# aerius-labs/indexed-merkle-tree-halo2

Measured on AMD Instinct MI355X. Metric: indexed-tree insertions/sec at depth=32 (bn256::Fr), higher is better.
Workload: dtype u32 limbs (9 x 29-bit, Montgomery mod p), 64-bit accumulate

## Files before the change

indexed-merkle-tree-halo2_amd/csrc/imt_consts.hpp:

```cpp
#pragma once
#include <cstdint>

namespace imt {
namespace dev {

constexpr int NL = 9;
constexpr uint32_t MASK29 = (1u << 29) - 1;

struct Fe {
    uint32_t v[NL];
};

constexpr int RF = 8, RP = 57;
struct PoseidonConsts {
    Fe rc_full[RF][3];
    Fe rc_h2p2[3];
    Fe k_partial[RP];
    Fe mats[2][3][3];
    Fe sp_row[RP][3];
    Fe sp_col[RP][2];
    Fe sp_gamma[RP];
    Fe cap0;
    Fe one;
    Fe from_canon;
    Fe from_mont256;
    Fe to_mont256;
    Fe int_one;
    Fe zero_leaf;
};

struct TraceConsts {
    Fe absorb[3][3];
    Fe full_c[RF][3];
    Fe partial[RP];
    Fe mats[2][3][3];
    Fe row[RP][3];
    Fe col_hat[RP][2];
};
constexpr int TRACE_ROWS_H2 = 1208, TRACE_ROWS_H3 = 1209;

}
}
```

indexed-merkle-tree-halo2_amd/csrc/imt_coop_device.hpp:

```cpp
#pragma once
#if !defined(__HIP_DEVICE_COMPILE__)
#error "device-only header"
#endif
#include <cstddef>
#include "imt_device.hpp"

namespace imt {
namespace dev {
namespace coop {

constexpr unsigned TAB_DWORDS = sizeof(PoseidonConsts) / 4;
#define IMT_COOP_E(member) ((unsigned)(offsetof(PoseidonConsts, member) / sizeof(Fe)))

__device__ __forceinline__ void tab_fill(uint32_t* tab, const PoseidonConsts& pc) {
    const uint32_t* src = reinterpret_cast<const uint32_t*>(&pc);
    for (unsigned i = threadIdx.x; i < TAB_DWORDS; i += blockDim.x) tab[i] = src[i];
    __syncthreads();
}
__device__ __forceinline__ void tab_fe(Fe& r, const uint32_t* tab, unsigned entry) {
#pragma unroll
    for (int i = 0; i < NL; i++) r.v[i] = tab[entry * NL + i];
}
template <int J>
__device__ __forceinline__ void quad_bcast(Fe& r, const Fe& x) {
#pragma unroll
    for (int i = 0; i < NL; i++) r.v[i] = (uint32_t)__builtin_amdgcn_mov_dpp((int)x.v[i], J * 0x55, 0xf, 0xf, true);
}
__device__ __forceinline__ void sel(Fe& r, bool c, const Fe& a, const Fe& b) {
#pragma unroll
    for (int i = 0; i < NL; i++) r.v[i] = c ? a.v[i] : b.v[i];
}

__device__ __forceinline__ void permute(const uint32_t* tab, Fe& S, unsigned ri, unsigned first_rc) {
    const bool is0 = ri == 0;
#pragma unroll 1
    for (int st = 0; st < RF + RP; st++) {
        if (st < RF / 2 || st >= RF / 2 + RP) {
            const int f = st < RF / 2 ? st : st - RP;
            Fe k, v, x2, x4, y, Y[3], M[3];
            tab_fe(k, tab, (st == 0 ? first_rc : IMT_COOP_E(rc_full) + 3u * (unsigned)f) + ri);
            add_lazy(v, S, k);
            masm::sqr_v_narrow(x2, v);
            masm::sqr_v_narrow(x4, x2);
            masm::mul_vv_narrow(y, &x4, &v);
            quad_bcast<0>(Y[0], y);
// ... 57 lines not shown
```

indexed-merkle-tree-halo2_amd/csrc/imt_device.hpp:

```cpp
#pragma once
#include <cstddef>
#include <cstdint>
#include "imt_consts.hpp"

#if defined(__HIPCC__)
#include <hip/hip_runtime.h>
#define IMT_HD __host__ __device__ __forceinline__
#else
#define IMT_HD inline
#endif

namespace imt {
namespace dev {

#define IMT_P29_0 0x10000001u
#define IMT_P29_1 0x1f0fac9fu
#define IMT_P29_2 0x0e5c2450u
#define IMT_P29_3 0x07d090f3u
#define IMT_P29_4 0x1585d283u
#define IMT_P29_5 0x02db40c0u
#define IMT_P29_6 0x00a6e141u
#define IMT_P29_7 0x0e5c2634u
#define IMT_P29_8 0x0030644eu
constexpr uint32_t N0INV29 = 0x0fffffffu;
// ... 158 lines not shown
    for (int i = 0; i < NL; i++) {
        uint32_t d = a.v[i] - p29(i) - borrow;
        borrow = (i < NL - 1) ? (d >> 31) : 0;
        a.v[i] = (i < NL - 1) ? (d & MASK29) : d;
    }
}

template <int SH>
IMT_HD constexpr uint32_t p29_shl(int i) {
    return i == 0 ? ((p29(0) << SH) & MASK29)
         : i < NL - 1 ? (((p29(i) << SH) | (p29(i - 1) >> (29 - SH))) & MASK29)
                      : ((p29(i) << SH) | (p29(i - 1) >> (29 - SH)));
}
template <int SH>
IMT_HD void cond_sub_p_shl(Fe& a) {
    bool ge = true;
#pragma unroll
    for (int i = 0; i < NL; i++) {
        const uint32_t pi = p29_shl<SH>(i);
        if (a.v[i] != pi) ge = a.v[i] > pi;
    }
    if (ge) {
        uint32_t borrow = 0;
#pragma unroll
        for (int i = 0; i < NL; i++) {
            uint32_t d = a.v[i] - p29_shl<SH>(i) - borrow;
            borrow = (i < NL - 1) ? (d >> 31) : 0;
            a.v[i] = (i < NL - 1) ? (d & MASK29) : d;
        }
    }
}

IMT_HD void canonicalize(Fe& a) {
    cond_sub_p_shl<3>(a);
    cond_sub_p_shl<2>(a);
    cond_sub_p_shl<1>(a);
    cond_sub_p_shl<0>(a);
}

IMT_HD void unpack(Fe& r, const uint32_t w[8]) {
#pragma unroll
    for (int i = 0; i < NL; i++) {
        const int bit = 29 * i, wi = bit >> 5, sh = bit & 31;
        uint32_t lo = w[wi] >> sh;
        if (sh > 3 && wi + 1 < 8) lo |= w[wi + 1] << (32 - sh);
        r.v[i] = lo & MASK29;
    }
}
IMT_HD void pack(uint32_t w[8], const Fe& a) {
#pragma unroll
    for (int j = 0; j < 8; j++) {
        const int lo_limb = (32 * j) / 29, off = 32 * j - 29 * lo_limb;
        uint32_t x = a.v[lo_limb] >> off;
        const int have = 29 - off;
        if (have < 32 && lo_limb + 1 < NL) x |= a.v[lo_limb + 1] << have;
        if (have + 29 < 32 && lo_limb + 2 < NL) x |= a.v[lo_limb + 2] << (have + 29);
        w[j] = x;
    }
}

struct alignas(16) Word4 { uint32_t x, y, z, w; };
IMT_HD void load_packed(Fe& r, const void* ptr) {
    const Word4* q = reinterpret_cast<const Word4*>(ptr);
    Word4 x = q[0], y = q[1];
    uint32_t w[8] = {x.x, x.y, x.z, x.w, y.x, y.y, y.z, y.w};
    unpack(r, w);
}
IMT_HD void store_packed(void* ptr, const Fe& a) {
    uint32_t w[8];
    pack(w, a);
    Word4* q = reinterpret_cast<Word4*>(ptr);
    q[0] = Word4{w[0], w[1], w[2], w[3]};
    q[1] = Word4{w[4], w[5], w[6], w[7]};
}



IMT_HD void sbox(Fe& x) {
    Fe x2, x4;
    mont_sqr(x2, x);
    mont_sqr(x4, x2);
    mont_mul(x, x4, x);
}

IMT_HD void permute(const PoseidonConsts& pc, Fe s[3], const Fe* first_rc) {
    constexpr int NSTEP = RF + (RP + 1) / 2;
#pragma unroll 1
    for (int st = 0; st < NSTEP; st++) {
        if (st < RF / 2 || st >= RF / 2 + (RP + 1) / 2) {
            const int fr = st < RF / 2 ? st : st - (RP + 1) / 2;
            const Fe* rc = (st == 0) ? first_rc : pc.rc_full[fr];
            add_lazy(s[0], s[0], rc[0]);
            add_lazy(s[1], s[1], rc[1]);
            add_lazy(s[2], s[2], rc[2]);
            sbox(s[0]); sbox(s[1]); sbox(s[2]);
            const Fe(*mat)[3] = pc.mats[st == RF / 2 - 1 ? 1 : 0];
            Fe n0, n1, n2;
            mont_dot_uc<3, false>(n0, mat[0], s, s[0]);
            mont_dot_uc<3, false>(n1, mat[1], s, s[0]);
            mont_dot_uc<3, false>(n2, mat[2], s, s[0]);
            s[0] = n0; s[1] = n1; s[2] = n2;
        } else {
            const int p = 2 * (st - RF / 2);
            const bool second = p + 1 < RP;
            Fe v[4], y[2], n0;
            add_lazy(v[0], s[0], pc.k_partial[p]);
            sbox(v[0]);
            v[1] = s[1]; v[2] = s[2];
            mont_dot_uc<3, false>(n0, pc.sp_row[p], v, v[0]);
            y[0] = v[0];
#pragma unroll
            for (int i = 0; i < NL; i++) y[1].v[i] = 0;
            if (second) {
                add_lazy(v[0], n0, pc.k_partial[p + 1]);
                sbox(v[0]);
                v[3] = y[0];
                const Fe c4[4] = {pc.sp_row[p + 1][0], pc.sp_row[p + 1][1], pc.sp_row[p + 1][2], pc.sp_gamma[p + 1]};
                mont_dot_uc<4, false>(n0, c4, v, v[0]);
                y[1] = v[0];
            }
            const int q = second ? p + 1 : p;
            const Fe c1[2] = {pc.sp_col[p][0], pc.sp_col[q][0]};
            const Fe c2[2] = {pc.sp_col[p][1], pc.sp_col[q][1]};
            mont_dot_uc<2, true, false>(s[1], c1, y, s[1]);
            mont_dot_uc<2, true, false>(s[2], c2, y, s[2]);
            s[0] = n0;
        }
    }
}

IMT_HD void hash23(const PoseidonConsts& pc, Fe& out, const Fe& a, const Fe& b, const Fe& c, bool three) {
    Fe s[3] = {pc.cap0, a, b};
#pragma unroll 1
    for (int blk = 0; blk < 2; blk++) {
        const Fe* rc0 = pc.rc_full[0];
        if (blk == 1) {
            if (three) {
                add_lazy(s[1], s[1], c);
                add_lazy(s[2], s[2], pc.one);
                normalize(s[1]);
                normalize(s[2]);
            } else {
                rc0 = pc.rc_h2p2;
            }
        }
        permute(pc, s, rc0);
    }
    out = s[1];
    canonicalize(out);
}
IMT_HD void hash23_stashed(const PoseidonConsts& pc, Fe& out, const Fe& a, const Fe& b, bool three,
                           const uint32_t* stash, unsigned stride) {
    Fe s[3] = {pc.cap0, a, b};
#pragma unroll 1
    for (int blk = 0; blk < 2; blk++) {
        const Fe* rc0 = pc.rc_full[0];
        if (blk == 1) {
            if (three) {
// ... 54 lines not shown
```

indexed-merkle-tree-halo2_amd/csrc/imt_flags.hip:

```cpp
#include <hip/hip_runtime.h>
#include <algorithm>
#include "imt_flags.hpp"

namespace {

__global__ void k_flag_set(uint64_t* flag, uint64_t value) {
    if (threadIdx.x == 0 && blockIdx.x == 0) __hip_atomic_store(flag, value, __ATOMIC_RELEASE, __HIP_MEMORY_SCOPE_SYSTEM);
}

__device__ inline bool poisoned(const uint32_t* poison) {
    return poison && __hip_atomic_load(poison, __ATOMIC_RELAXED, __HIP_MEMORY_SCOPE_SYSTEM) != 0;
}

__global__ void k_flag_set_checked(uint64_t* flag, uint64_t value, const uint32_t* poison) {
    if (threadIdx.x == 0 && blockIdx.x == 0 && !poisoned(poison)) __hip_atomic_store(flag, value, __ATOMIC_RELEASE, __HIP_MEMORY_SCOPE_SYSTEM);
}

__global__ void k_flag_wait(imt::launch::FlagWait w) {
    if (threadIdx.x != 0 || blockIdx.x != 0) return;
    if (poisoned(w.err)) return;
    const uint64_t t0 = wall_clock64();
    for (int i = 0; i < w.n; i++) {
        while (__hip_atomic_load(w.flag[i], __ATOMIC_ACQUIRE, __HIP_MEMORY_SCOPE_SYSTEM) < w.value) {
            if (wall_clock64() - t0 > w.timeout_ticks) {
                __hip_atomic_fetch_or(w.err, 1u << (i & 31), __ATOMIC_RELAXED, __HIP_MEMORY_SCOPE_SYSTEM);
                return;
            }
            __builtin_amdgcn_s_sleep(64);
        }
    }
}

__global__ void k_copy16(uint4* __restrict__ dst, const uint4* __restrict__ src, size_t n16, const uint32_t* poison) {
    if (poisoned(poison)) return;
    for (size_t i = (size_t)blockIdx.x * blockDim.x + threadIdx.x; i < n16; i += (size_t)gridDim.x * blockDim.x) dst[i] = src[i];
}

__global__ void k_copy16_multi(imt::launch::CopyJobs jobs, size_t n16, const uint32_t* poison) {
    if (poisoned(poison)) return;
    uint4* __restrict__ dst = (uint4*)jobs.dst[blockIdx.y];
    const uint4* __restrict__ src = (const uint4*)jobs.src[blockIdx.y];
    for (size_t i = (size_t)blockIdx.x * blockDim.x + threadIdx.x; i < n16; i += (size_t)gridDim.x * blockDim.x) dst[i] = src[i];
}

__global__ void k_spin(uint64_t ticks, uint64_t* end_stamp) {
    if (threadIdx.x != 0 || blockIdx.x != 0) return;
    const uint64_t t0 = wall_clock64();
    while (wall_clock64() - t0 < ticks) __builtin_amdgcn_s_sleep(32);
    *end_stamp = wall_clock64();
}
__global__ void k_stamp(uint64_t* stamp) {
    if (threadIdx.x == 0 && blockIdx.x == 0) *stamp = wall_clock64();
}

}

namespace imt {
namespace launch {

void copy16(hipStream_t s, void* dst, const void* src, size_t bytes, const uint32_t* poison) {
    const size_t n16 = bytes / 16;
    if (!n16) return;
    const unsigned blocks = (unsigned)std::min<size_t>((n16 + 255) / 256, 512);
    hipLaunchKernelGGL(k_copy16, dim3(blocks), dim3(256), 0, s, (uint4*)dst, (const uint4*)src, n16, poison);
}

void copy16_multi(hipStream_t s, const CopyJobs& jobs, size_t bytes, const uint32_t* poison) {
    const size_t n16 = bytes / 16;
    if (!n16 || jobs.n <= 0) return;
    const unsigned blocks = (unsigned)std::min<size_t>((n16 + 255) / 256, 64);
    hipLaunchKernelGGL(k_copy16_multi, dim3(blocks, (unsigned)jobs.n), dim3(256), 0, s, jobs, n16, poison);
}

void flag_set_checked(hipStream_t s, uint64_t* flag, uint64_t value, const uint32_t* poison) {
    hipLaunchKernelGGL(k_flag_set_checked, dim3(1), dim3(64), 0, s, flag, value, poison);
}

void spin(hipStream_t s, uint64_t ticks, uint64_t* end_stamp) { hipLaunchKernelGGL(k_spin, dim3(1), dim3(64), 0, s, ticks, end_stamp); }
void stamp(hipStream_t s, uint64_t* out) { hipLaunchKernelGGL(k_stamp, dim3(1), dim3(64), 0, s, out); }

void flag_set(hipStream_t s, uint64_t* flag, uint64_t value) { hipLaunchKernelGGL(k_flag_set, dim3(1), dim3(64), 0, s, flag, value); }

void flag_wait(hipStream_t s, const FlagWait& w) {
    if (w.n > 0) hipLaunchKernelGGL(k_flag_wait, dim3(1), dim3(64), 0, s, w);
}

}
}
```

indexed-merkle-tree-halo2_amd/csrc/imt_flags.hpp:

```cpp
#pragma once
#include <hip/hip_runtime_api.h>
#include <cstdint>

namespace imt {
namespace launch {

constexpr int FLAG_WAIT_MAX = 16;
struct FlagWait {
    const uint64_t* flag[FLAG_WAIT_MAX];
    int n;
    uint64_t value;
    uint64_t timeout_ticks;
    uint32_t* err;
};
void flag_set(hipStream_t s, uint64_t* flag, uint64_t value);
void flag_wait(hipStream_t s, const FlagWait& w);
void copy16(hipStream_t s, void* dst, const void* src, size_t bytes, const uint32_t* poison = nullptr);
struct CopyJobs {
    void* dst[FLAG_WAIT_MAX];
    const void* src[FLAG_WAIT_MAX];
    int n;
};
void copy16_multi(hipStream_t s, const CopyJobs& jobs, size_t bytes, const uint32_t* poison);
void flag_set_checked(hipStream_t s, uint64_t* flag, uint64_t value, const uint32_t* poison);
void spin(hipStream_t s, uint64_t ticks, uint64_t* end_stamp);
void stamp(hipStream_t s, uint64_t* out);

}
}
```

indexed-merkle-tree-halo2_amd/csrc/imt_fr_host.hpp:

```cpp
#pragma once
#include <cstdint>
#include <cstring>

namespace imt {

typedef unsigned __int128 u128;

struct HFr {
    uint64_t l[4];
    bool operator==(const HFr& o) const { return std::memcmp(l, o.l, 32) == 0; }
};

struct HField {
    static constexpr uint64_t P[4] = {0x43e1f593f0000001ULL, 0x2833e84879b97091ULL,
                                      0xb85045b68181585dULL, 0x30644e72e131a029ULL};
    uint64_t inv;
    HFr r1, r2;
    HFr r3;

    HField() {
        uint64_t x = 1;
        for (int i = 0; i < 7; i++) x *= 2 - P[0] * x;
        inv = 0 - x;
        uint64_t t[4] = {1, 0, 0, 0};
// ... 66 lines not shown
        for (int i = 0; i < 4; i++) {
            uint64_t m = t[i] * inv;
            u128 c = 0;
            for (int j = 0; j < 4; j++) {
                c += (u128)m * P[j] + t[i + j];
                t[i + j] = (uint64_t)c;
                c >>= 64;
            }
            for (int k = i + 4; k < 9 && c; k++) {
                c += t[k];
                t[k] = (uint64_t)c;
                c >>= 64;
            }
        }
        HFr o;
        std::memcpy(o.l, t + 4, 32);
        if (t[8] || geq_p(o.l)) sub_p(o.l);
        return o;
    }
    HFr from_u64(uint64_t v) const { return mul(HFr{{v, 0, 0, 0}}, r2); }
    HFr zero() const { return HFr{{0, 0, 0, 0}}; }
    HFr one() const { return r1; }
    bool from_bytes(HFr& out, const uint8_t in[32]) const {
        HFr t;
        std::memcpy(t.l, in, 32);
        if (geq_p(t.l)) return false;
        out = mul(t, r2);
        return true;
    }
    void to_bytes(uint8_t out[32], const HFr& a) const {
        HFr t = mul(a, HFr{{1, 0, 0, 0}});
        std::memcpy(out, t.l, 32);
    }
    HFr inverse(const HFr& a) const {
        uint64_t e[4] = {P[0] - 2, P[1], P[2], P[3]};
        HFr acc = r1, base = a;
        for (int i = 0; i < 256; i++) {
            if ((e[i / 64] >> (i % 64)) & 1) acc = mul(acc, base);
            base = mul(base, base);
        }
        return acc;
    }
    bool is_zero(const HFr& a) const { return (a.l[0] | a.l[1] | a.l[2] | a.l[3]) == 0; }
};

inline int cmp_le32(const uint8_t* a, const uint8_t* b) {
    const uint64_t* x = reinterpret_cast<const uint64_t*>(a);
    const uint64_t* y = reinterpret_cast<const uint64_t*>(b);
    uint64_t xa[4], ya[4];
    std::memcpy(xa, x, 32);
    std::memcpy(ya, y, 32);
    for (int i = 3; i >= 0; i--) {
        if (xa[i] != ya[i]) return xa[i] < ya[i] ? -1 : 1;
    }
    return 0;
}

}
```

indexed-merkle-tree-halo2_amd/csrc/imt_params.cpp:

```cpp
#include "imt_params.hpp"

namespace imt {

namespace {
struct Grain {
    uint8_t b[80];
    int pos = 0;
    int new_bit() {
        int p = pos;
        auto g = [&](int k) { return b[(p + k) % 80]; };
        int nb = g(62) ^ g(51) ^ g(38) ^ g(23) ^ g(13) ^ g(0);
        b[p] = (uint8_t)nb;
        pos = (p + 1) % 80;
        return nb;
    }
    int next() {
        while (!new_bit()) new_bit();
        return new_bit();
    }
    void take254(uint8_t le[32]) {
        std::memset(le, 0, 32);
        for (int i = 253; i >= 0; i--)
            if (next()) le[i / 8] |= (uint8_t)(1u << (i % 8));
    }
// ... 20 lines not shown

void HostPoseidon::permute_opt(HFr s[3]) const {
    auto sbox = [&](HFr& x) {
        HFr x2 = F.mul(x, x), x4 = F.mul(x2, x2);
        x = F.mul(x4, x);
    };
    auto dense = [&](const HFr m[3][3]) {
        HFr n[3];
        for (int i = 0; i < 3; i++) {
            n[i] = F.mul(m[i][0], s[0]);
            n[i] = F.add(n[i], F.mul(m[i][1], s[1]));
            n[i] = F.add(n[i], F.mul(m[i][2], s[2]));
        }
        s[0] = n[0]; s[1] = n[1]; s[2] = n[2];
    };
    for (int r = 0; r < 65; r++) {
        if (r < 4 || r >= 61) {
            const int fr = r < 4 ? r : r - 57;
            for (int i = 0; i < 3; i++) s[i] = F.add(s[i], rc_full[fr][i]);
            for (int i = 0; i < 3; i++) sbox(s[i]);
            dense(r == 3 ? pre : mds);
        } else {
            const int p = r - 4;
            HFr y = F.add(s[0], k_partial[p]);
            sbox(y);
            HFr n0 = F.mul(sp_row[p][0], y);
            n0 = F.add(n0, F.mul(sp_row[p][1], s[1]));
            n0 = F.add(n0, F.mul(sp_row[p][2], s[2]));
            s[1] = F.add(s[1], F.mul(sp_col[p][0], y));
            s[2] = F.add(s[2], F.mul(sp_col[p][1], y));
            s[0] = n0;
        }
    }
}

void HostPoseidon::permute_spec(HFr s[3]) const {
    auto x5c = [&](HFr& x, const HFr& c) {
        HFr x2 = F.mul(x, x), x4 = F.mul(x2, x2);
        x = F.add(F.mul(x4, x), c);
    };
    auto dense = [&](const HFr m[3][3]) {
        HFr n[3];
        for (int i = 0; i < 3; i++) {
            n[i] = F.mul(m[i][0], s[0]);
            n[i] = F.add(n[i], F.mul(m[i][1], s[1]));
            n[i] = F.add(n[i], F.mul(m[i][2], s[2]));
        }
        s[0] = n[0]; s[1] = n[1]; s[2] = n[2];
    };
    for (int i = 0; i < 3; i++) s[i] = F.add(s[i], tr_start[0][i]);
    for (int r = 1; r <= 4; r++) {
        for (int i = 0; i < 3; i++) x5c(s[i], tr_start[r][i]);
        dense(r == 4 ? tr_pre : mds);
    }
    for (int p = 0; p < 57; p++) {
        x5c(s[0], tr_partial[p]);
        HFr n0 = F.mul(tr_row[p][0], s[0]);
        n0 = F.add(n0, F.mul(tr_row[p][1], s[1]));
        n0 = F.add(n0, F.mul(tr_row[p][2], s[2]));
        s[1] = F.add(F.mul(tr_col_hat[p][0], s[0]), s[1]);
        s[2] = F.add(F.mul(tr_col_hat[p][1], s[0]), s[2]);
        s[0] = n0;
    }
    for (int r = 0; r < 4; r++) {
        for (int i = 0; i < 3; i++) x5c(s[i], r < 3 ? tr_end[r][i] : F.zero());
        dense(mds);
// ... 66 lines not shown
        HFr mw[3];
        matvec(mds, w, mw);
        for (int i = 0; i < 3; i++) rc_full[4][i] = F.add(rc[61][i], mw[i]);
    }
    for (int r = 62; r < 65; r++)
        for (int i = 0; i < 3; i++) rc_full[r - 57][i] = rc[r][i];

    HFr cur[3][3];
    std::memcpy(cur, mds, sizeof cur);
    for (int p = 60; p >= 4; p--) {
        HFr det = F.sub(F.mul(cur[1][1], cur[2][2]), F.mul(cur[1][2], cur[2][1]));
        if (F.is_zero(det)) { err = "singular MDS sub-block"; return false; }
        HFr di = F.inverse(det);
        HFr Dinv[2][2] = {{F.mul(cur[2][2], di), F.mul(F.sub(F.zero(), cur[1][2]), di)},
                          {F.mul(F.sub(F.zero(), cur[2][1]), di), F.mul(cur[1][1], di)}};
        sp_row[p - 4][0] = cur[0][0];
        sp_row[p - 4][1] = F.add(F.mul(cur[0][1], Dinv[0][0]), F.mul(cur[0][2], Dinv[1][0]));
        sp_row[p - 4][2] = F.add(F.mul(cur[0][1], Dinv[0][1]), F.mul(cur[0][2], Dinv[1][1]));
        sp_col[p - 4][0] = cur[1][0];
        sp_col[p - 4][1] = cur[2][0];
        HFr np[3][3] = {{F.one(), F.zero(), F.zero()},
                        {F.zero(), cur[1][1], cur[1][2]},
                        {F.zero(), cur[2][1], cur[2][2]}};
        HFr nxt[3][3];
        for (int i = 0; i < 3; i++)
            for (int j = 0; j < 3; j++) {
                nxt[i][j] = F.mul(np[i][0], mds[0][j]);
                nxt[i][j] = F.add(nxt[i][j], F.mul(np[i][1], mds[1][j]));
                nxt[i][j] = F.add(nxt[i][j], F.mul(np[i][2], mds[2][j]));
            }
        std::memcpy(cur, nxt, sizeof cur);
    }
    std::memcpy(pre, cur, sizeof pre);

    {
        typedef HFr M3[3][3];
        auto mat_mul = [&](const M3 a, const M3 b, M3 o) {
            HFr r[3][3];
            for (int i = 0; i < 3; i++)
                for (int j = 0; j < 3; j++) {
                    r[i][j] = F.mul(a[i][0], b[0][j]);
                    r[i][j] = F.add(r[i][j], F.mul(a[i][1], b[1][j]));
                    r[i][j] = F.add(r[i][j], F.mul(a[i][2], b[2][j]));
                }
            std::memcpy(o, r, sizeof r);
        };
        HFr minv[3][3];
        {
            auto cof = [&](int r0, int r1, int c0, int c1) {
                return F.sub(F.mul(mds[r0][c0], mds[r1][c1]), F.mul(mds[r0][c1], mds[r1][c0]));
            };
            HFr adj[3][3];
            for (int i = 0; i < 3; i++)
                for (int j = 0; j < 3; j++) {
                    const int r0 = (j + 1) % 3, r1 = (j + 2) % 3, c0 = (i + 1) % 3, c1 = (i + 2) % 3;
                    adj[i][j] = cof(r0, r1, c0, c1);
                }
            HFr det = F.add(F.add(F.mul(mds[0][0], adj[0][0]), F.mul(mds[0][1], adj[1][0])), F.mul(mds[0][2], adj[2][0]));
            if (F.is_zero(det)) { err = "singular MDS"; return false; }
            HFr di = F.inverse(det);
            for (int i = 0; i < 3; i++)
                for (int j = 0; j < 3; j++) minv[i][j] = F.mul(adj[i][j], di);
        }
        for (int i = 0; i < 3; i++) tr_start[0][i] = rc[0][i];
        for (int r = 1; r < 4; r++) matvec(minv, rc[r], tr_start[r]);
        HFr acc[3] = {rc[61][0], rc[61][1], rc[61][2]};
        for (int p = 56; p >= 0; p--) {
            HFr tmp[3];
            matvec(minv, acc, tmp);
            tr_partial[p] = tmp[0];
            acc[0] = rc[4 + p][0];
            acc[1] = F.add(tmp[1], rc[4 + p][1]);
            acc[2] = F.add(tmp[2], rc[4 + p][2]);
        }
        matvec(minv, acc, tr_start[4]);
        for (int r = 0; r < 3; r++) matvec(minv, rc[62 + r], tr_end[r]);
        HFr mt[3][3], a[3][3];
        for (int i = 0; i < 3; i++)
            for (int j = 0; j < 3; j++) mt[i][j] = a[i][j] = mds[j][i];
        for (int k = 0; k < 57; k++) {
            const int p = 56 - k;
            HFr det = F.sub(F.mul(a[1][1], a[2][2]), F.mul(a[1][2], a[2][1]));
            if (F.is_zero(det)) { err = "singular MDS minor"; return false; }
            HFr di = F.inverse(det);
            HFr hi[2][2] = {{F.mul(a[2][2], di), F.mul(F.sub(F.zero(), a[1][2]), di)},
                            {F.mul(F.sub(F.zero(), a[2][1]), di), F.mul(a[1][1], di)}};
            tr_row[p][0] = a[0][0];
            tr_row[p][1] = F.add(F.mul(hi[0][0], a[1][0]), F.mul(hi[0][1], a[2][0]));
            tr_row[p][2] = F.add(F.mul(hi[1][0], a[1][0]), F.mul(hi[1][1], a[2][0]));
            tr_col_hat[p][0] = a[0][1];
            tr_col_hat[p][1] = a[0][2];
            HFr prime[3][3] = {{F.one(), F.zero(), F.zero()}, {F.zero(), a[1][1], a[1][2]}, {F.zero(), a[2][1], a[2][2]}};
            mat_mul(mt, prime, a);
        }
        for (int i = 0; i < 3; i++)
            for (int j = 0; j < 3; j++) tr_pre[i][j] = a[j][i];
    }

    for (uint64_t t = 0; t < 4; t++) {
        HFr a[3] = {F.from_u64(t * 7919), F.from_u64(t * t + 1), F.mul(cap0, F.from_u64(t + 3))};
        HFr b[3] = {a[0], a[1], a[2]};
        permute_plain(a);
        permute_opt(b);
        if (!(a[0] == b[0] && a[1] == b[1] && a[2] == b[2])) {
            err = "optimised Poseidon schedule disagrees with the plain form";
            return false;
        }
        HFr c3[3] = {F.from_u64(t * 7919), F.from_u64(t * t + 1), F.mul(cap0, F.from_u64(t + 3))};
        permute_spec(c3);
        if (!(a[0] == c3[0] && a[1] == c3[1] && a[2] == c3[2])) {
            err = "halo2-base form of the Poseidon schedule disagrees with the plain form";
            return false;
        }
    }
    return true;
}

void HostPoseidon::fill_trace_consts(dev::TraceConsts& tc) const {
    for (int i = 0; i < 3; i++) {
        tc.absorb[0][i] = to_dev(tr_start[0][i]);
        tc.absorb[1][i] = to_dev(i == 2 ? F.add(tr_start[0][i], F.one()) : tr_start[0][i]);
        tc.absorb[2][i] = to_dev(i == 1 ? F.add(tr_start[0][i], F.one()) : tr_start[0][i]);
    }
    for (int f = 0; f < 8; f++)
        for (int i = 0; i < 3; i++)
            tc.full_c[f][i] = to_dev(f < 4 ? tr_start[f + 1][i] : f < 7 ? tr_end[f - 4][i] : F.zero());
    for (int p = 0; p < 57; p++) {
        tc.partial[p] = to_dev(tr_partial[p]);
        for (int i = 0; i < 3; i++) tc.row[p][i] = to_dev(tr_row[p][i]);
        for (int i = 0; i < 2; i++) tc.col_hat[p][i] = to_dev(tr_col_hat[p][i]);
    }
    for (int i = 0; i < 3; i++)
        for (int j = 0; j < 3; j++) {
            tc.mats[0][i][j] = to_dev(mds[i][j]);
            tc.mats[1][i][j] = to_dev(tr_pre[i][j]);
        }
}

dev::Fe HostPoseidon::int_to_dev_limbs(const uint8_t le[32]) const {
    dev::Fe o;
    for (int i = 0; i < dev::NL; i++) {
        uint32_t v = 0;
        for (int k = 0; k < 29; k++) {
            int bit = 29 * i + k;
            if (bit < 256 && ((le[bit / 8] >> (bit % 8)) & 1)) v |= 1u << k;
        }
        o.v[i] = v;
    }
    return o;
}

dev::Fe HostPoseidon::to_dev(const HFr& x) const {
    HFr two29 = F.from_u64(1ULL << 29);
    HFr t = x;
    for (int i = 0; i < 9; i++) t = F.mul(t, two29);
    uint8_t le[32];
    F.to_bytes(le, t);
    return int_to_dev_limbs(le);
}

void HostPoseidon::fill_consts(dev::PoseidonConsts& pc) const {
    for (int r = 0; r < 8; r++)
        for (int i = 0; i < 3; i++) pc.rc_full[r][i] = to_dev(rc_full[r][i]);
    pc.rc_h2p2[0] = to_dev(rc_full[0][0]);
    pc.rc_h2p2[1] = to_dev(F.add(rc_full[0][1], F.one()));
    pc.rc_h2p2[2] = to_dev(rc_full[0][2]);
    pc.sp_gamma[0] = to_dev(F.zero());
    for (int p = 1; p < 57; p++)
        pc.sp_gamma[p] = to_dev(F.add(F.mul(sp_row[p][1], sp_col[p - 1][0]), F.mul(sp_row[p][2], sp_col[p - 1][1])));
    for (int p = 0; p < 57; p++) {
        pc.k_partial[p] = to_dev(k_partial[p]);
        for (int i = 0; i < 3; i++) pc.sp_row[p][i] = to_dev(sp_row[p][i]);
        for (int i = 0; i < 2; i++) pc.sp_col[p][i] = to_dev(sp_col[p][i]);
    }
    for (int i = 0; i < 3; i++)
        for (int j = 0; j < 3; j++) {
            pc.mats[0][i][j] = to_dev(mds[i][j]);
            pc.mats[1][i][j] = to_dev(pre[i][j]);
        }
    pc.cap0 = to_dev(cap0);
    pc.one = to_dev(F.one());
    HFr two29 = F.from_u64(1ULL << 29), r261 = F.one();
    for (int i = 0; i < 9; i++) r261 = F.mul(r261, two29);
    HFr two64 = cap0, two256 = F.mul(F.mul(two64, two64), F.mul(two64, two64));
    uint8_t le[32];
    auto as_int = [&](const HFr& x) { F.to_bytes(le, x); return int_to_dev_limbs(le); };
    pc.from_canon = as_int(F.mul(r261, r261));
    pc.from_mont256 = as_int(F.mul(F.mul(r261, r261), F.inverse(two256)));
    pc.to_mont256 = as_int(two256);
    std::memset(le, 0, 32); le[0] = 1;
    pc.int_one = int_to_dev_limbs(le);
    HFr z = F.zero();
    pc.zero_leaf = to_dev(hash3(z, z, z));
}

}
```

indexed-merkle-tree-halo2_amd/csrc/imt_params.hpp:

```cpp
#pragma once
#include "imt_consts.hpp"
#include "imt_fr_host.hpp"
#include <string>
#include <vector>

namespace imt {

struct HostPoseidon {
    HField F;
    HFr rc[65][3];
    HFr mds[3][3];
    HFr rc_full[8][3];
    HFr k_partial[57];
    HFr pre[3][3];
    HFr sp_row[57][3];
    HFr sp_col[57][2];
    HFr cap0;
    HFr tr_start[5][3], tr_partial[57], tr_end[3][3];
    HFr tr_pre[3][3];
    HFr tr_row[57][3], tr_col_hat[57][2];

    bool init(std::string& err);

    void permute_plain(HFr s[3]) const;
    void permute_opt(HFr s[3]) const;
    void permute_spec(HFr s[3]) const;
    void fill_trace_consts(dev::TraceConsts& tc) const;
    HFr hash2(const HFr& a, const HFr& b) const;
    HFr hash3(const HFr& a, const HFr& b, const HFr& c) const;

    dev::Fe to_dev(const HFr& x) const;
    dev::Fe int_to_dev_limbs(const uint8_t le[32]) const;
    void fill_consts(dev::PoseidonConsts& pc) const;
};

}
```

indexed-merkle-tree-halo2_amd/csrc/imt_sliced.cpp:

```cpp
#include <fcntl.h>
#include <sys/mman.h>
#include <sys/stat.h>
#include <unistd.h>
#include <algorithm>
#include <atomic>
#include <chrono>
#include <condition_variable>
#include <deque>
#include <mutex>
#include <cstdio>
#include <cstring>
#include <memory>
#include <new>
#include <string>
#include <thread>
#include <vector>
#include "imt_flags.hpp"
#include "imt_itree_internal.hpp"
#include "imt_sliced_sched.hpp"
#include "imt_sliced_transport.hpp"

using namespace imt::sliced;

namespace {
// ... 60 lines not shown
        }
    };
    env("IMT_SLICED_COMM_STREAMS", IMT_SLICED_OPT_COMM_STREAMS, o);
    env("IMT_SLICED_COMM_PRIO", IMT_SLICED_OPT_COMM_PRIORITY, o);
    env("IMT_SLICED_ROUND_PRIO", IMT_SLICED_OPT_ROUND_PRIORITIES, o);
    env("IMT_SLICED_APPLY_STREAMS", IMT_SLICED_OPT_APPLY_STREAMS, o);
    env("IMT_SLICED_PREP_STREAM", IMT_SLICED_OPT_PREP_STREAM, o);
    env("IMT_SLICED_VERIFY_QUEUES", IMT_SLICED_OPT_VERIFY_QUEUES, o);
    env("IMT_SLICED_WATCHDOG_MS", IMT_SLICED_OPT_WATCHDOG_MS, o);
    env("IMT_SLICED_TIMING", IMT_SLICED_OPT_TIMING, o);
    env("IMT_SLICED_COMM_PLACEMENT", IMT_SLICED_OPT_COMM_PLACEMENT, o);
    env("IMT_SLICED_POOLS", IMT_SLICED_OPT_POOLS, o);
    return o;
}

template <class Query>
int bounded_wait(imt_ctx* ctx, long limit_ms, Query query, const char* what) {
    const auto t0 = std::chrono::steady_clock::now();
    for (unsigned spins = 0;; spins++) {
        const hipError_t e = query();
        if (e == hipSuccess) return IMT_OK;
        if (e != hipErrorNotReady) return ctx->hip_fail(e, what);
        if (spins > 2000) std::this_thread::sleep_for(std::chrono::microseconds(50));
        if (limit_ms > 0 && (spins & 63) == 63 &&
            std::chrono::duration<double, std::milli>(std::chrono::steady_clock::now() - t0).count() > (double)limit_ms)
            return ctx->fail(IMT_ERR_TIMEOUT, "gave up after %ld ms waiting for %s (IMT_SLICED_OPT_WATCHDOG_MS)", limit_ms, what);
    }
}

struct QueueProbe {
    imt_ctx* ctx = nullptr;
    uint64_t* d = nullptr;
    static constexpr int MAXS = 16;
    uint64_t spin_ticks = 20000;
    int probes = 0;

    int init(imt_ctx* c) {
        ctx = c;
        int khz = 100000;
        if (hipDeviceGetAttribute(&khz, hipDeviceAttributeWallClockRate, c->device) != hipSuccess || khz <= 0) khz = 100000;
        spin_ticks = (uint64_t)khz / 5;
        IMT_HIP(c, hipMalloc((void**)&d, sizeof(uint64_t) * (MAXS + 1)));
        imt::launch::spin(c->stream, 1, d + MAXS);
        imt::launch::stamp(c->stream, d);
        IMT_HIP(c, hipStreamSynchronize(c->stream));
        return IMT_OK;
    }
    ~QueueProbe() {
        if (d) hipFree(d);
    }
    int run(hipStream_t busy, const hipStream_t* others, int n, char* behind) {
        if (n > MAXS) return ctx->fail(IMT_ERR_INTERNAL, "queue probe: too many streams");
        uint64_t h[MAXS + 1];
        IMT_HIP(ctx, hipStreamSynchronize(busy));
        for (int j = 0; j < n; j++) IMT_HIP(ctx, hipStreamSynchronize(others[j]));
        IMT_HIP(ctx, hipMemsetAsync(d, 0, sizeof(uint64_t) * (MAXS + 1), ctx->stream));
        IMT_HIP(ctx, hipStreamSynchronize(ctx->stream));
        imt::launch::spin(busy, spin_ticks, d + MAXS);
        for (int j = 0; j < n; j++) imt::launch::stamp(others[j], d + j);
        IMT_HIP(ctx, hipGetLastError());
        IMT_HIP(ctx, hipStreamSynchronize(busy));
        for (int j = 0; j < n; j++) IMT_HIP(ctx, hipStreamSynchronize(others[j]));
        IMT_HIP(ctx, hipMemcpy(h, d, sizeof h, hipMemcpyDeviceToHost));
        for (int j = 0; j < n; j++) behind[j] = h[j] >= h[MAXS];
        probes++;
        return IMT_OK;
    }
};

struct HipBackend : Backend {
    imt_itree* tree;
    imt_ctx* ctx;
    hipStream_t rs[ROUNDS] = {}, cs[ROUNDS] = {}, aps[ROUNDS] = {};
    int n_comm = ROUNDS;
    int round_prio = 0;
    SlicedOptions opt;
    int q_round[ROUNDS], q_comm[ROUNDS], q_apply[ROUNDS];
    int n_queues = 0, placement = IMT_SLICED_PLACEMENT_UNVERIFIED, streams_recreated = 0;
    bool comm_own_queues = false;
    bool hung = false;
    std::string placement_note;

    explicit HipBackend(imt_itree* t) : tree(t), ctx(imt_itree_ctx(t)) {
        for (int i = 0; i < ROUNDS; i++) q_round[i] = q_comm[i] = q_apply[i] = -1;
    }
    int new_stream(hipStream_t* out, int prio) {
        IMT_HIP(ctx, hipStreamCreateWithPriority(out, hipStreamNonBlocking, prio));
        return IMT_OK;
    }
    void adopt(hipStream_t s) { ctx->side_streams.push_back(s); }
    int init(const SlicedOptions& o, int channels) {
        opt = o;
// ... 1146 lines not shown
```

Baseline: 3.018 million.

## Rescale Poseidon constants by fifth roots to turn multiplies into additions

Precomputes fifth-root diagonal rescalings of the Poseidon state on the host, so that row 0 of most full-round matrices becomes (1,1,1) and one sparse-column coefficient becomes 1. The device permute then uses additions instead of Montgomery dot products for those entries, with a periodic fold to keep the lazily reduced limbs bounded and an extra canonicalize step. The queue probe is also changed to end its spin once all stamp kernels have run, which cuts probe wait time while raising the maximum spin. The rescaled path is checked against the plain schedule on extra inputs, but the lazy-reduction bounds are a correctness risk.

```diff
diff --git a/indexed-merkle-tree-halo2_amd/csrc/imt_consts.hpp b/indexed-merkle-tree-halo2_amd/csrc/imt_consts.hpp
--- a/indexed-merkle-tree-halo2_amd/csrc/imt_consts.hpp
+++ b/indexed-merkle-tree-halo2_amd/csrc/imt_consts.hpp
@@ -19,7 +19,6 @@
     Fe mats[2][3][3];
     Fe sp_row[RP][3];
     Fe sp_col[RP][2];
-    Fe sp_gamma[RP];
     Fe cap0;
     Fe one;
     Fe from_canon;
@@ -27,6 +26,12 @@
     Fe to_mont256;
     Fe int_one;
     Fe zero_leaf;
+    Fe sc_rc[RF][3];
+    Fe sc_mats[RF][3][3];
+    Fe sc_k[RP];
+    Fe sc_row[RP][3];
+    Fe sc_gamma[RP];
+    Fe sc_u[RP];
 };
 
 struct TraceConsts {
diff --git a/indexed-merkle-tree-halo2_amd/csrc/imt_coop_device.hpp b/indexed-merkle-tree-halo2_amd/csrc/imt_coop_device.hpp
--- a/indexed-merkle-tree-halo2_amd/csrc/imt_coop_device.hpp
+++ b/indexed-merkle-tree-halo2_amd/csrc/imt_coop_device.hpp
@@ -9,8 +9,9 @@
 namespace dev {
 namespace coop {
 
-constexpr unsigned TAB_DWORDS = sizeof(PoseidonConsts) / 4;
+constexpr unsigned TAB_DWORDS = offsetof(PoseidonConsts, sc_rc) / 4;
 #define IMT_COOP_E(member) ((unsigned)(offsetof(PoseidonConsts, member) / sizeof(Fe)))
+static_assert(TAB_DWORDS * 4 <= 16236, "the coop kernels' LDS table must not grow");
 
 __device__ __forceinline__ void tab_fill(uint32_t* tab, const PoseidonConsts& pc) {
     const uint32_t* src = reinterpret_cast<const uint32_t*>(&pc);
diff --git a/indexed-merkle-tree-halo2_amd/csrc/imt_device.hpp b/indexed-merkle-tree-halo2_amd/csrc/imt_device.hpp
--- a/indexed-merkle-tree-halo2_amd/csrc/imt_device.hpp
+++ b/indexed-merkle-tree-halo2_amd/csrc/imt_device.hpp
@@ -214,6 +214,7 @@
 }
 
 IMT_HD void canonicalize(Fe& a) {
+    cond_sub_p_shl<4>(a);
     cond_sub_p_shl<3>(a);
     cond_sub_p_shl<2>(a);
     cond_sub_p_shl<1>(a);
@@ -265,47 +266,68 @@
     mont_mul(x, x4, x);
 }
 
+IMT_HD constexpr uint32_t pc29(int i) { return i == 0 ? (1u << 29) - p29(0) : MASK29 - p29(i); }
+constexpr uint32_t FOLD_RECIP = 1354;
+
+IMT_HD void fold_p(Fe& a) {
+    const uint32_t q = (uint32_t)(((uint64_t)a.v[NL - 1] * FOLD_RECIP) >> 32);
+    uint64_t acc = 0;
+#pragma unroll
+    for (int i = 0; i < NL; i++) {
+        acc = (acc >> 29) + a.v[i] + (uint64_t)q * pc29(i);
+        a.v[i] = i < NL - 1 ? (uint32_t)acc & MASK29 : (uint32_t)(acc - ((uint64_t)q << 29));
+    }
+}
+
 IMT_HD void permute(const PoseidonConsts& pc, Fe s[3], const Fe* first_rc) {
     constexpr int NSTEP = RF + (RP + 1) / 2;
 #pragma unroll 1
     for (int st = 0; st < NSTEP; st++) {
         if (st < RF / 2 || st >= RF / 2 + (RP + 1) / 2) {
             const int fr = st < RF / 2 ? st : st - (RP + 1) / 2;
-            const Fe* rc = (st == 0) ? first_rc : pc.rc_full[fr];
+            const Fe* rc = (st == 0) ? first_rc : pc.sc_rc[fr];
             add_lazy(s[0], s[0], rc[0]);
             add_lazy(s[1], s[1], rc[1]);
             add_lazy(s[2], s[2], rc[2]);
             sbox(s[0]); sbox(s[1]); sbox(s[2]);
-            const Fe(*mat)[3] = pc.mats[st == RF / 2 - 1 ? 1 : 0];
+            const Fe(*mat)[3] = pc.sc_mats[fr];
             Fe n0, n1, n2;
-            mont_dot_uc<3, false>(n0, mat[0], s, s[0]);
+            if (fr == 0 || fr == RF / 2) {
+                mont_dot_uc<3, false>(n0, mat[0], s, s[0]);
+            } else {
+                add_lazy(n0, s[0], s[1]);
+                add_lazy(n0, n0, s[2]);
+                normalize(n0);
+            }
             mont_dot_uc<3, false>(n1, mat[1], s, s[0]);
             mont_dot_uc<3, false>(n2, mat[2], s, s[0]);
             s[0] = n0; s[1] = n1; s[2] = n2;
         } else {
             const int p = 2 * (st - RF / 2);
             const bool second = p + 1 < RP;
-            Fe v[4], y[2], n0;
-            add_lazy(v[0], s[0], pc.k_partial[p]);
+            Fe v[4], z[2], n0;
+            add_lazy(v[0], s[0], pc.sc_k[p]);
             sbox(v[0]);
             v[1] = s[1]; v[2] = s[2];
-            mont_dot_uc<3, false>(n0, pc.sp_row[p], v, v[0]);
-            y[0] = v[0];
-#pragma unroll
-            for (int i = 0; i < NL; i++) y[1].v[i] = 0;
+            mont_dot_uc<3, false>(n0, pc.sc_row[p], v, v[0]);
+            z[0] = v[0];
+#pragma unroll
+            for (int i = 0; i < NL; i++) z[1].v[i] = 0;
             if (second) {
-                add_lazy(v[0], n0, pc.k_partial[p + 1]);
+                add_lazy(v[0], n0, pc.sc_k[p + 1]);
                 sbox(v[0]);
-                v[3] = y[0];
-                const Fe c4[4] = {pc.sp_row[p + 1][0], pc.sp_row[p + 1][1], pc.sp_row[p + 1][2], pc.sp_gamma[p + 1]};
+                v[3] = z[0];
+                const Fe c4[4] = {pc.sc_row[p + 1][0], pc.sc_row[p + 1][1], pc.sc_row[p + 1][2], pc.sc_gamma[p + 1]};
                 mont_dot_uc<4, false>(n0, c4, v, v[0]);
-                y[1] = v[0];
+                z[1] = v[0];
             }
             const int q = second ? p + 1 : p;
-            const Fe c1[2] = {pc.sp_col[p][0], pc.sp_col[q][0]};
-            const Fe c2[2] = {pc.sp_col[p][1], pc.sp_col[q][1]};
-            mont_dot_uc<2, true, false>(s[1], c1, y, s[1]);
-            mont_dot_uc<2, true, false>(s[2], c2, y, s[2]);
+            const Fe cu[2] = {pc.sc_u[p], pc.sc_u[q]};
+            mont_dot_uc<2, true, false>(s[2], cu, z, s[2]);
+            add_lazy(s[1], s[1], z[0]);
+            add_lazy(s[1], s[1], z[1]);
+            normalize(s[1]);
+            if ((p & 7) == 6) fold_p(s[1]);
             s[0] = n0;
         }
     }
diff --git a/indexed-merkle-tree-halo2_amd/csrc/imt_flags.hip b/indexed-merkle-tree-halo2_amd/csrc/imt_flags.hip
--- a/indexed-merkle-tree-halo2_amd/csrc/imt_flags.hip
+++ b/indexed-merkle-tree-halo2_amd/csrc/imt_flags.hip
@@ -43,14 +43,18 @@
     for (size_t i = (size_t)blockIdx.x * blockDim.x + threadIdx.x; i < n16; i += (size_t)gridDim.x * blockDim.x) dst[i] = src[i];
 }
 
-__global__ void k_spin(uint64_t ticks, uint64_t* end_stamp) {
+__global__ void k_spin(uint64_t ticks, uint64_t* end_stamp, const uint64_t* count, uint64_t n) {
     if (threadIdx.x != 0 || blockIdx.x != 0) return;
     const uint64_t t0 = wall_clock64();
-    while (wall_clock64() - t0 < ticks) __builtin_amdgcn_s_sleep(32);
+    while (wall_clock64() - t0 < ticks && __hip_atomic_load(count, __ATOMIC_ACQUIRE, __HIP_MEMORY_SCOPE_AGENT) < n)
+        __builtin_amdgcn_s_sleep(32);
     *end_stamp = wall_clock64();
 }
-__global__ void k_stamp(uint64_t* stamp) {
-    if (threadIdx.x == 0 && blockIdx.x == 0) *stamp = wall_clock64();
+__global__ void k_stamp(uint64_t* stamp, uint64_t* count) {
+    if (threadIdx.x == 0 && blockIdx.x == 0) {
+        *stamp = wall_clock64();
+        __hip_atomic_fetch_add(count, (uint64_t)1, __ATOMIC_RELEASE, __HIP_MEMORY_SCOPE_AGENT);
+    }
 }
 
 }
@@ -76,8 +80,10 @@
     hipLaunchKernelGGL(k_flag_set_checked, dim3(1), dim3(64), 0, s, flag, value, poison);
 }
 
-void spin(hipStream_t s, uint64_t ticks, uint64_t* end_stamp) { hipLaunchKernelGGL(k_spin, dim3(1), dim3(64), 0, s, ticks, end_stamp); }
-void stamp(hipStream_t s, uint64_t* out) { hipLaunchKernelGGL(k_stamp, dim3(1), dim3(64), 0, s, out); }
+void spin(hipStream_t s, uint64_t ticks, uint64_t* end_stamp, const uint64_t* count, uint64_t n) {
+    hipLaunchKernelGGL(k_spin, dim3(1), dim3(64), 0, s, ticks, end_stamp, count, n);
+}
+void stamp(hipStream_t s, uint64_t* out, uint64_t* count) { hipLaunchKernelGGL(k_stamp, dim3(1), dim3(64), 0, s, out, count); }
 
 void flag_set(hipStream_t s, uint64_t* flag, uint64_t value) { hipLaunchKernelGGL(k_flag_set, dim3(1), dim3(64), 0, s, flag, value); }
 
diff --git a/indexed-merkle-tree-halo2_amd/csrc/imt_flags.hpp b/indexed-merkle-tree-halo2_amd/csrc/imt_flags.hpp
--- a/indexed-merkle-tree-halo2_amd/csrc/imt_flags.hpp
+++ b/indexed-merkle-tree-halo2_amd/csrc/imt_flags.hpp
@@ -23,8 +23,8 @@
 };
 void copy16_multi(hipStream_t s, const CopyJobs& jobs, size_t bytes, const uint32_t* poison);
 void flag_set_checked(hipStream_t s, uint64_t* flag, uint64_t value, const uint32_t* poison);
-void spin(hipStream_t s, uint64_t ticks, uint64_t* end_stamp);
-void stamp(hipStream_t s, uint64_t* out);
+void spin(hipStream_t s, uint64_t ticks, uint64_t* end_stamp, const uint64_t* count, uint64_t n);
+void stamp(hipStream_t s, uint64_t* out, uint64_t* count);
 
 }
 }
diff --git a/indexed-merkle-tree-halo2_amd/csrc/imt_fr_host.hpp b/indexed-merkle-tree-halo2_amd/csrc/imt_fr_host.hpp
--- a/indexed-merkle-tree-halo2_amd/csrc/imt_fr_host.hpp
+++ b/indexed-merkle-tree-halo2_amd/csrc/imt_fr_host.hpp
@@ -122,14 +122,33 @@
         HFr t = mul(a, HFr{{1, 0, 0, 0}});
         std::memcpy(out, t.l, 32);
     }
-    HFr inverse(const HFr& a) const {
-        uint64_t e[4] = {P[0] - 2, P[1], P[2], P[3]};
+    HFr pow(const HFr& a, const uint64_t e[4]) const {
         HFr acc = r1, base = a;
         for (int i = 0; i < 256; i++) {
             if ((e[i / 64] >> (i % 64)) & 1) acc = mul(acc, base);
             base = mul(base, base);
         }
         return acc;
+    }
+    HFr inverse(const HFr& a) const {
+        const uint64_t e[4] = {P[0] - 2, P[1], P[2], P[3]};
+        return pow(a, e);
+    }
+    HFr fifth_root(const HFr& a) const {
+        uint64_t e[4];
+        u128 c = 1;
+        for (int i = 0; i < 4; i++) {
+            c += (u128)P[i] * 4 - (i == 0 ? 4 : 0);
+            e[i] = (uint64_t)c;
+            c >>= 64;
+        }
+        u128 rem = 0;
+        for (int i = 3; i >= 0; i--) {
+            u128 cur = (rem << 64) | e[i];
+            e[i] = (uint64_t)(cur / 5);
+            rem = cur % 5;
+        }
+        return pow(a, e);
     }
     bool is_zero(const HFr& a) const { return (a.l[0] | a.l[1] | a.l[2] | a.l[3]) == 0; }
 };
diff --git a/indexed-merkle-tree-halo2_amd/csrc/imt_params.cpp b/indexed-merkle-tree-halo2_amd/csrc/imt_params.cpp
--- a/indexed-merkle-tree-halo2_amd/csrc/imt_params.cpp
+++ b/indexed-merkle-tree-halo2_amd/csrc/imt_params.cpp
@@ -76,6 +76,44 @@
             s[0] = n0;
         }
     }
+}
+
+void HostPoseidon::permute_scaled(HFr s[3]) const {
+    auto sbox = [&](HFr& x) {
+        HFr x2 = F.mul(x, x), x4 = F.mul(x2, x2);
+        x = F.mul(x4, x);
+    };
+    auto dot = [&](const HFr* c, const HFr* v, int n) {
+        HFr o = F.zero();
+        for (int i = 0; i < n; i++) o = F.add(o, F.mul(c[i], v[i]));
+        return o;
+    };
+    auto full = [&](int f) {
+        for (int i = 0; i < 3; i++) s[i] = F.add(s[i], sc_rc[f][i]);
+        for (int i = 0; i < 3; i++) sbox(s[i]);
+        const HFr n0 = (f == 0 || f == 4) ? dot(sc_mats[f][0], s, 3) : F.add(F.add(s[0], s[1]), s[2]);
+        const HFr n1 = dot(sc_mats[f][1], s, 3), n2 = dot(sc_mats[f][2], s, 3);
+        s[0] = n0; s[1] = n1; s[2] = n2;
+    };
+    for (int f = 0; f < 4; f++) full(f);
+    for (int p = 0; p < 57; p += 2) {
+        HFr z0 = F.add(s[0], sc_k[p]);
+        sbox(z0);
+        const HFr v3[3] = {z0, s[1], s[2]};
+        HFr n0 = dot(sc_row[p], v3, 3), z1 = F.zero();
+        if (p + 1 < 57) {
+            z1 = F.add(n0, sc_k[p + 1]);
+            sbox(z1);
+            const HFr c4[4] = {sc_row[p + 1][0], sc_row[p + 1][1], sc_row[p + 1][2], sc_gamma[p + 1]};
+            const HFr v4[4] = {z1, s[1], s[2], z0};
+            n0 = dot(c4, v4, 4);
+        }
+        s[1] = F.add(s[1], F.add(z0, z1));
+        s[2] = F.add(s[2], F.mul(sc_u[p], z0));
+        if (p + 1 < 57) s[2] = F.add(s[2], F.mul(sc_u[p + 1], z1));
+        s[0] = n0;
+    }
+    for (int f = 4; f < 8; f++) full(f);
 }
 
 void HostPoseidon::permute_spec(HFr s[3]) const {
@@ -208,6 +246,58 @@
         std::memcpy(cur, nxt, sizeof cur);
     }
     std::memcpy(pre, cur, sizeof pre);
+
+    {
+        HFr lam[58];
+        for (int p = 0; p < 57; p++) {
+            if (F.is_zero(sp_col[p][0])) { err = "sparse column entry col[p][0] is zero: no fifth-root rescaling"; return false; }
+            lam[p] = F.fifth_root(F.inverse(sp_col[p][0]));
+            HFr l2 = F.mul(lam[p], lam[p]);
+            if (!(F.mul(F.mul(l2, l2), F.mul(lam[p], sp_col[p][0])) == F.one())) { err = "fifth root check failed"; return false; }
+        }
+        lam[57] = F.one();
+        for (int p = 0; p < 57; p++) {
+            const HFr li = F.inverse(lam[p]), ln = F.inverse(lam[p + 1]);
+            sc_k[p] = F.mul(k_partial[p], li);
+            sc_row[p][0] = F.mul(sp_row[p][0], F.mul(F.inverse(sp_col[p][0]), ln));
+            sc_row[p][1] = F.mul(sp_row[p][1], ln);
+            sc_row[p][2] = F.mul(sp_row[p][2], ln);
+            sc_u[p] = F.mul(sp_col[p][1], F.inverse(sp_col[p][0]));
+        }
+        sc_gamma[0] = F.zero();
+        for (int p = 1; p < 57; p++) sc_gamma[p] = F.add(sc_row[p][1], F.mul(sc_row[p][2], sc_u[p - 1]));
+
+        HFr d[9][3];
+        for (int i = 0; i < 3; i++) d[0][i] = d[4][i] = d[8][i] = F.one();
+        const HFr d4in[3] = {lam[0], F.one(), F.one()};
+        auto solve = [&](int f, const HFr m[3][3], const HFr& dn0) {
+            for (int j = 0; j < 3; j++) {
+                if (F.is_zero(m[0][j])) { err = "zero entry in row 0 of a full-round matrix"; return false; }
+                d[f][j] = F.fifth_root(F.mul(dn0, F.inverse(m[0][j])));
+            }
+            return true;
+        };
+        for (int f = 7; f >= 5; f--)
+            if (!solve(f, mds, d[f + 1][0])) return false;
+        if (!solve(3, pre, d4in[0])) return false;
+        for (int f = 2; f >= 1; f--)
+            if (!solve(f, mds, d[f + 1][0])) return false;
+        for (int f = 0; f < 8; f++) {
+            const HFr(*m)[3] = f == 3 ? pre : mds;
+            const HFr* dn = f == 3 ? d4in : d[f + 1];
+            for (int i = 0; i < 3; i++) {
+                sc_rc[f][i] = F.mul(rc_full[f][i], F.inverse(d[f][i]));
+                const HFr dni = F.inverse(dn[i]);
+                for (int j = 0; j < 3; j++) {
+                    HFr d2 = F.mul(d[f][j], d[f][j]);
+                    sc_mats[f][i][j] = F.mul(F.mul(m[i][j], dni), F.mul(F.mul(d2, d2), d[f][j]));
+                }
+            }
+            if (f != 0 && f != 4)
+                for (int j = 0; j < 3; j++)
+                    if (!(sc_mats[f][0][j] == F.one())) { err = "rescaled full-round row 0 is not (1, 1, 1)"; return false; }
+        }
+    }
 
     {
         typedef HFr M3[3][3];
@@ -273,16 +363,22 @@
             for (int j = 0; j < 3; j++) tr_pre[i][j] = a[j][i];
     }
 
-    for (uint64_t t = 0; t < 4; t++) {
+    for (uint64_t t = 0; t < 6; t++) {
         HFr a[3] = {F.from_u64(t * 7919), F.from_u64(t * t + 1), F.mul(cap0, F.from_u64(t + 3))};
-        HFr b[3] = {a[0], a[1], a[2]};
+        if (t == 4) a[0] = a[1] = a[2] = F.sub(F.zero(), F.one());
+        if (t == 5) a[0] = a[1] = a[2] = F.mul(cap0, cap0);
+        HFr b[3] = {a[0], a[1], a[2]}, sc[3] = {a[0], a[1], a[2]}, c3[3] = {a[0], a[1], a[2]};
         permute_plain(a);
         permute_opt(b);
+        permute_scaled(sc);
         if (!(a[0] == b[0] && a[1] == b[1] && a[2] == b[2])) {
             err = "optimised Poseidon schedule disagrees with the plain form";
             return false;
         }
-        HFr c3[3] = {F.from_u64(t * 7919), F.from_u64(t * t + 1), F.mul(cap0, F.from_u64(t + 3))};
+        if (!(a[0] == sc[0] && a[1] == sc[1] && a[2] == sc[2])) {
+            err = "rescaled Poseidon schedule disagrees with the plain form";
+            return false;
+        }
         permute_spec(c3);
         if (!(a[0] == c3[0] && a[1] == c3[1] && a[2] == c3[2])) {
             err = "halo2-base form of the Poseidon schedule disagrees with the plain form";
@@ -341,14 +437,20 @@
     pc.rc_h2p2[0] = to_dev(rc_full[0][0]);
     pc.rc_h2p2[1] = to_dev(F.add(rc_full[0][1], F.one()));
     pc.rc_h2p2[2] = to_dev(rc_full[0][2]);
-    pc.sp_gamma[0] = to_dev(F.zero());
-    for (int p = 1; p < 57; p++)
-        pc.sp_gamma[p] = to_dev(F.add(F.mul(sp_row[p][1], sp_col[p - 1][0]), F.mul(sp_row[p][2], sp_col[p - 1][1])));
     for (int p = 0; p < 57; p++) {
         pc.k_partial[p] = to_dev(k_partial[p]);
         for (int i = 0; i < 3; i++) pc.sp_row[p][i] = to_dev(sp_row[p][i]);
         for (int i = 0; i < 2; i++) pc.sp_col[p][i] = to_dev(sp_col[p][i]);
-    }
+        pc.sc_k[p] = to_dev(sc_k[p]);
+        for (int i = 0; i < 3; i++) pc.sc_row[p][i] = to_dev(sc_row[p][i]);
+        pc.sc_gamma[p] = to_dev(sc_gamma[p]);
+        pc.sc_u[p] = to_dev(sc_u[p]);
+    }
+    for (int f = 0; f < 8; f++)
+        for (int i = 0; i < 3; i++) {
+            pc.sc_rc[f][i] = to_dev(sc_rc[f][i]);
+            for (int j = 0; j < 3; j++) pc.sc_mats[f][i][j] = to_dev(sc_mats[f][i][j]);
+        }
     for (int i = 0; i < 3; i++)
         for (int j = 0; j < 3; j++) {
             pc.mats[0][i][j] = to_dev(mds[i][j]);
diff --git a/indexed-merkle-tree-halo2_amd/csrc/imt_params.hpp b/indexed-merkle-tree-halo2_amd/csrc/imt_params.hpp
--- a/indexed-merkle-tree-halo2_amd/csrc/imt_params.hpp
+++ b/indexed-merkle-tree-halo2_amd/csrc/imt_params.hpp
@@ -16,6 +16,9 @@
     HFr sp_row[57][3];
     HFr sp_col[57][2];
     HFr cap0;
+    HFr sc_rc[8][3];
+    HFr sc_mats[8][3][3];
+    HFr sc_k[57], sc_row[57][3], sc_gamma[57], sc_u[57];
     HFr tr_start[5][3], tr_partial[57], tr_end[3][3];
     HFr tr_pre[3][3];
     HFr tr_row[57][3], tr_col_hat[57][2];
@@ -24,6 +27,7 @@
 
     void permute_plain(HFr s[3]) const;
     void permute_opt(HFr s[3]) const;
+    void permute_scaled(HFr s[3]) const;
     void permute_spec(HFr s[3]) const;
     void fill_trace_consts(dev::TraceConsts& tc) const;
     HFr hash2(const HFr& a, const HFr& b) const;
diff --git a/indexed-merkle-tree-halo2_amd/csrc/imt_sliced.cpp b/indexed-merkle-tree-halo2_amd/csrc/imt_sliced.cpp
--- a/indexed-merkle-tree-halo2_amd/csrc/imt_sliced.cpp
+++ b/indexed-merkle-tree-halo2_amd/csrc/imt_sliced.cpp
@@ -116,17 +116,18 @@
     imt_ctx* ctx = nullptr;
     uint64_t* d = nullptr;
     static constexpr int MAXS = 16;
-    uint64_t spin_ticks = 20000;
+    uint64_t spin_ticks = 5000000;
     int probes = 0;
 
     int init(imt_ctx* c) {
         ctx = c;
         int khz = 100000;
         if (hipDeviceGetAttribute(&khz, hipDeviceAttributeWallClockRate, c->device) != hipSuccess || khz <= 0) khz = 100000;
-        spin_ticks = (uint64_t)khz / 5;
-        IMT_HIP(c, hipMalloc((void**)&d, sizeof(uint64_t) * (MAXS + 1)));
-        imt::launch::spin(c->stream, 1, d + MAXS);
-        imt::launch::stamp(c->stream, d);
+        spin_ticks = (uint64_t)khz * 50;
+        IMT_HIP(c, hipMalloc((void**)&d, sizeof(uint64_t) * (MAXS + 2)));
+        IMT_HIP(c, hipMemsetAsync(d, 0, sizeof(uint64_t) * (MAXS + 2), c->stream));
+        imt::launch::spin(c->stream, 1, d + MAXS, d + MAXS + 1, 0);
+        imt::launch::stamp(c->stream, d, d + MAXS + 1);
         IMT_HIP(c, hipStreamSynchronize(c->stream));
         return IMT_OK;
     }
@@ -138,10 +139,10 @@
         uint64_t h[MAXS + 1];
         IMT_HIP(ctx, hipStreamSynchronize(busy));
         for (int j = 0; j < n; j++) IMT_HIP(ctx, hipStreamSynchronize(others[j]));
-        IMT_HIP(ctx, hipMemsetAsync(d, 0, sizeof(uint64_t) * (MAXS + 1), ctx->stream));
+        IMT_HIP(ctx, hipMemsetAsync(d, 0, sizeof(uint64_t) * (MAXS + 2), ctx->stream));
         IMT_HIP(ctx, hipStreamSynchronize(ctx->stream));
-        imt::launch::spin(busy, spin_ticks, d + MAXS);
-        for (int j = 0; j < n; j++) imt::launch::stamp(others[j], d + j);
+        imt::launch::spin(busy, spin_ticks, d + MAXS, d + MAXS + 1, (uint64_t)n);
+        for (int j = 0; j < n; j++) imt::launch::stamp(others[j], d + j, d + MAXS + 1);
         IMT_HIP(ctx, hipGetLastError());
         IMT_HIP(ctx, hipStreamSynchronize(busy));
         for (int j = 0; j < n; j++) IMT_HIP(ctx, hipStreamSynchronize(others[j]));
```

After: 3.355 million (median of 6 runs). 1.11x the previous value.
